# oxfordcontrol/Clarabel.rs

Hardware: AMD Instinct MI355X
Metric: IPM iterations/sec (KKT factor+solve) at n=10^6 SOCP, 1/2/4/8 GPUs (higher is better)
Workload: dtype f64

## Files before the change

### clarabel.rs_amd/csrc/bundle_ir.hip

```cpp
#include "dev_common.hpp"
#include "bundle_symv.hpp"
#include "ir_refine.hpp"
#include "grid_sync.hpp"

namespace chip {
namespace dev {

namespace {

constexpr int IR_SH_FWD = 3, IR_SH_BWD = 3, IR_SH_SYMV = 3;
constexpr int IR_RPT = 2;
constexpr int IR_FATCAP = 256;

template <bool FWDMODE, int SH, int RPT, int TW>
__device__ __forceinline__ void bundle_sweep_cols(const LdlView &v, const BundleView &bv, int b, double *xs,
                                                  const double *xt, double *tacc, int k, int *fat, int &nfat,
                                                  const double *__restrict__ dinv = nullptr) {
    constexpr int CH = RPT * TW;
    const int s0 = bv.bundle_ptr[b], nloc = bv.bundle_ptr[b + 1] - s0;
    const int *lv = bv.blvl + bv.blvl_ptr[b];
    const int nl = bv.blvl_ptr[b + 1] - bv.blvl_ptr[b] - 1;
    const int lane = threadIdx.x & 63, wv = threadIdx.x >> 6;
    if (FWDMODE && (int)threadIdx.x < 8) tacc[threadIdx.x] = 0.0;
    double tpart = 0.0;
// ... 174 lines not shown
    int i[FLAT_U], j[FLAT_U];
    double v[FLAT_U];
};
__device__ __forceinline__ void flat_batch_clear(FlatBatch &fb) {
#pragma unroll
    for (int u = 0; u < FLAT_U; ++u) fb.i[u] = -1, fb.j[u] = 0, fb.v[u] = 0.0;
}
template <bool FWDMODE, int TW>
__device__ __forceinline__ void flat_request_first(const LdlView &v, const int *lev_e, int nl, int dl, int tid, FlatBatch &fb) {
    int step = 0, base = 0, ee = 0;
    while (step < nl) {
        const int l = FWDMODE ? step : nl - 1 - step;
        base = lev_e[l];
        ee = lev_e[l + 1];
        if (base < ee) break;
        ++step;
    }
    if (step < nl) {
#pragma unroll
        for (int u = 0; u < FLAT_U; ++u) {
            const int t = base + u * TW + tid;
            const bool ok = t < ee;
            const int tc = ok ? t : ee - 1;
            const int ri = (int)v.Li16[tc + dl], rj = (int)v.Lj16[tc + dl];
            const double rv = v.Lx[tc];
            fb.i[u] = ok ? ri : -1;
            fb.j[u] = ok ? rj : 0;
            fb.v[u] = ok ? rv : 0.0;
        }
    } else {
        flat_batch_clear(fb);
    }
}
template <bool FWDMODE, int TW, bool HAVE_FIRST = true>
__device__ __forceinline__ void bundle_sweep_flat_ahead(const LdlView &v, double *xs, const double *xt, double *tacc, int k,
                                                        const int *lev_e, int dl, int nloc, int nl, const FlatBatch &first) {
    static_assert(TW != 512, "two batches in flight: not within the 80 registers of the 512-thread form");
    int tid = threadIdx.x;
    asm volatile("" : "+v"(tid));
    const int lane = tid & 63;
    if (FWDMODE && tid < 8) tacc[tid] = 0.0;
    double tpart = 0.0;
    int step = 0, base = 0, ee = 0;
    auto level_range = [&](int st_, int &eb_, int &ee_) {
        const int l = FWDMODE ? st_ : nl - 1 - st_;
        eb_ = lev_e[l];
        ee_ = lev_e[l + 1];
    };
    lds_barrier();
    while (step < nl) {
        level_range(step, base, ee);
        if (base < ee) break;
        ++step;
    }
    int ci[FLAT_U], cj[FLAT_U], ni[FLAT_U], nj[FLAT_U];
    double cv[FLAT_U], nv[FLAT_U];
    auto request = [&](int bs, int en, int *ii, int *jj, double *vv) {
#pragma unroll
        for (int u = 0; u < FLAT_U; ++u) {
            const int t = bs + u * TW + tid;
            const bool ok = t < en;
            ii[u] = ok ? (int)v.Li16[t + dl] : -1;
            jj[u] = ok ? (int)v.Lj16[t + dl] : 0;
            vv[u] = ok ? v.Lx[t] : 0.0;
        }
    };
    if (HAVE_FIRST) {
#pragma unroll
        for (int u = 0; u < FLAT_U; ++u) {
            ci[u] = first.i[u];
            cj[u] = first.j[u];
            cv[u] = first.v[u];
        }
    } else if (step < nl) {
        request(base, ee, ci, cj, cv);
    }
    while (step < nl) {
        int nstep = step, nbase = base + TW * FLAT_U, nee = ee;
        if (nbase >= nee) {
            nstep = step + 1;
            while (nstep < nl) {
                level_range(nstep, nbase, nee);
                if (nbase < nee) break;
                ++nstep;
            }
        }
        if (nstep < nl) request(nbase, nee, ni, nj, nv);
#pragma unroll
        for (int u = 0; u < FLAT_U; ++u) {
            const int i = ci[u];
            if (i < 0) continue;
            if (FWDMODE) {
                const double val = cv[u] * xs[cj[u]];
                if (i < nloc) atomicAdd(&xs[i], -val);
                else if (k == 1) tpart += val;
                else atomicAdd(&tacc[i - nloc], val);
            } else {
                atomicAdd(&xs[cj[u]], -(cv[u] * (i < nloc ? xs[i] : xt[i - nloc])));
            }
        }
        if (nstep != step) lds_barrier();
        step = nstep;
        base = nbase;
        ee = nee;
#pragma unroll
        for (int u = 0; u < FLAT_U; ++u) {
            ci[u] = ni[u];
            cj[u] = nj[u];
            cv[u] = nv[u];
        }
    }
    if (FWDMODE && k == 1) {
        tpart = wave_sum_all(tpart);
        if (lane == 0 && tpart != 0.0) atomicAdd(&tacc[0], tpart);
    }
    lds_barrier();
}

template <bool FWDMODE, int TW>
__device__ __forceinline__ void bundle_sweep_flat(const LdlView &v, const BundleView &bv, int b, double *xs,
                                                  const double *xt, double *tacc, int k, const int *lev_e, int dl = 0) {
    const int s0 = bv.bundle_ptr[b], nloc = bv.bundle_ptr[b + 1] - s0;
    const int nl = bv.blvl_ptr[b + 1] - bv.blvl_ptr[b] - 1;
    int tid = threadIdx.x;
    asm volatile("" : "+v"(tid));
    if (!FWDMODE)
        for (int i = tid; i < nloc; i += TW) xs[i] *= v.Dinv[s0 + i];
    if constexpr (TW != 512) {
        bundle_sweep_flat_ahead<FWDMODE, TW, false>(v, xs, xt, tacc, k, lev_e, dl, nloc, nl, FlatBatch{});
    } else {
        const int lane = tid & 63;
// ... 617 lines not shown
        if ((GR ? gfirst : blockIdx.x == 0) && tid < k) {
            ir_put(ir, ir.perm[topnode(tid)], st.curt[tid]);
            cur[topnode(tid)] = st.curt[tid];
        }
    }
    if (GR && gfirst && tid == 0) {
        __hip_atomic_store(gf.gcnt + grp * 32, 0, __ATOMIC_RELAXED, __HIP_MEMORY_SCOPE_AGENT);
        __hip_atomic_store(gf.gcnt + grp * 32 + 1, 0, __ATOMIC_RELAXED, __HIP_MEMORY_SCOPE_AGENT);
    }
    if (blockIdx.x == 0 && tid == 0) {
        ir.res[0] = ok ? 1 : -1;
        ir.res[1] = st.rounds;
        ir.res[3] = st.sel;
        pub[64] = st.normb;
        pub[65] = st.norme;
    }
    stamp();
    ir_grid_exit(ir.ctl, __builtin_amdgcn_readfirstlane(st.gen) + 1, G);
}


constexpr int IRS_NPT = 12;
__device__ __forceinline__ int opaque_tid() {
    int t = threadIdx.x;
    asm volatile("" : "+v"(t));
    return t;
}

template <int TW, int NPT, int NLP>
__device__ __forceinline__ void irs_symv(const LdlView &v, const IrView &ir, const int *runs, const double (&c)[NPT],
                                         bool keep_e, double *xs, double *red, double *tacc3, int k, int s0,
                                         int nloc, int nleaf, const double *xt, double *out_norm, double *out_share,
                                         int du, bool have_fl, int fl_b, int fl_e, bool next_fwd,
                                         const int *lev_e, int nl, int dl, FlatBatch &nextb) {
    double cl[NLP];
    const int *__restrict__ Up = v.Up;
    const unsigned short *__restrict__ Ucol16 = v.Ucol16, *__restrict__ Urow16 = v.Urow16;
    const double *__restrict__ Ux = v.Ux;
    const int tid = opaque_tid();
    auto xpos = [&](int t) { return t < nleaf ? t : nloc + (t - nleaf); };
    constexpr int LR = 4, LS = 3;
    static_assert(NLP % LR == 0 && NLP <= NPT, "leaf passes");
    int tb[LR], te[LR];
#pragma unroll
    for (int u = 0; u < LR; ++u) {
        const int i = tid + u * TW;
        tb[u] = i < nleaf ? Up[s0 + i] : 0;
        te[u] = i < nleaf ? Up[s0 + i + 1] : 0;
    }
    const int fb = have_fl ? fl_b : Up[s0 + nleaf], fe = have_fl ? fl_e : Up[s0 + nloc];
    {
        RunWalk rw{runs, 0};
        double bq[NPT];
#pragma unroll
        for (int u = 0; u < NPT; ++u) {
            const int i = tid + u * TW;
            bq[u] = (i >= nleaf && i < nloc) ? ir_rhs(ir, rw.orig(i)) : 0.0;
        }
        lds_barrier();
#pragma unroll
        for (int u = 0; u < NPT; ++u) {
            const int i = tid + u * TW;
            if (i >= nleaf && i < nloc) {
                xs[xpos(i - nleaf)] = c[u];
                xs[i] = bq[u];
            }
        }
// ... 7 lines not shown
    lds_barrier();
    RunWalk rl{runs, 0};
#pragma unroll
    for (int p = 0; p < NLP / LR; ++p) {
        if (p * LR * TW < nleaf) {
            int jj[LR][LS];
            double vv[LR][LS], bi[LR], acc[LR];
#pragma unroll
            for (int u = 0; u < LR; ++u) {
                const int i = (p * LR + u) * TW + tid;
                bi[u] = i < nleaf ? ir_rhs(ir, rl.orig(i)) : 0.0;
                acc[u] = 0.0;
#pragma unroll
                for (int q = 0; q < LS; ++q) {
                    const int t = tb[u] + q;
                    const bool ok = t < te[u];
                    jj[u][q] = ok ? (int)Ucol16[t + du] : -1;
                    vv[u][q] = ok ? Ux[t] : 0.0;
                }
            }
#pragma unroll
            for (int u = 0; u < LR; ++u) {
                const int i = (p * LR + u) * TW + tid;
                const double xi = cl[p * LR + u];
                auto apply = [&](int j, double val) {
                    if (j >= nloc) {
                        acc[u] += val * xt[j - nloc];
                        if (k == 1) tpart += val * xi;
                        else atomicAdd(&tacc3[j - nloc], val * xi);
                    } else if (j == i) {
                        acc[u] += val * xi;
                    } else {
                        acc[u] += val * xs[xpos(j - nleaf)];
                        atomicAdd(&xs[j], -(val * xi));
                    }
                };
#pragma unroll
                for (int q = 0; q < LS; ++q)
                    if (jj[u][q] >= 0) apply(jj[u][q], vv[u][q]);
                for (int t = tb[u] + LS; t < te[u]; ++t) apply((int)Ucol16[t + du], Ux[t]);
                if (i < nleaf) {
                    const double val = bi[u] - acc[u];
                    if (keep_e) cl[p * LR + u] = val;
                    if (val != val) nan = true;
                    else mleaf = fmax(mleaf, fabs(val));
                }
                const int in = i + LR * TW;
                tb[u] = in < nleaf ? Up[s0 + in] : 0;
                te[u] = in < nleaf ? Up[s0 + in + 1] : 0;
            }
        }
    }
    {
        int fi[FLAT_U], fj[FLAT_U], ni[FLAT_U], nj[FLAT_U];
        double fv[FLAT_U], nv[FLAT_U];
        auto request = [&](int bs, int *pi, int *pj, double *pv) {
#pragma unroll
            for (int u = 0; u < FLAT_U; ++u) {
                const int t = bs + u * TW + tid;
                const bool ok = t < fe;
                pi[u] = ok ? (int)Urow16[t + du] : -1;
                pj[u] = ok ? (int)Ucol16[t + du] : 0;
                pv[u] = ok ? Ux[t] : 0.0;
            }
        };
        if (fb < fe) request(fb, fi, fj, fv);
        for (int base = fb; base < fe; base += TW * FLAT_U) {
            if (base + TW * FLAT_U < fe) request(base + TW * FLAT_U, ni, nj, nv);
            else {
#pragma unroll
                for (int u = 0; u < FLAT_U; ++u) ni[u] = -1;
            }
#pragma unroll
            for (int u = 0; u < FLAT_U; ++u) {
                const int i = fi[u], j = fj[u];
                if (i < 0) continue;
                const double xi = xs[xpos(i - nleaf)];
                if (j >= nloc) {
                    atomicAdd(&xs[i], -(fv[u] * xt[j - nloc]));
                    if (k == 1) tpart += fv[u] * xi;
                    else atomicAdd(&tacc3[j - nloc], fv[u] * xi);
                } else if (j == i) {
                    atomicAdd(&xs[i], -(fv[u] * xi));
                } else {
                    atomicAdd(&xs[i], -(fv[u] * xs[xpos(j - nleaf)]));
                    atomicAdd(&xs[j], -(fv[u] * xi));
                }
            }
#pragma unroll
            for (int u = 0; u < FLAT_U; ++u) {
                fi[u] = ni[u];
                fj[u] = nj[u];
                fv[u] = nv[u];
            }
        }
    }
    if (next_fwd) flat_request_first<true, TW>(v, lev_e, nl, dl, tid, nextb);
    lds_barrier();
    double m = mleaf;
#pragma unroll
    for (int u = 0; u < NPT; ++u) {
        const int i = tid + u * TW;
        if (i >= nleaf && i < nloc) {
            const double val = xs[i];
            if (val != val) nan = true;
            else m = fmax(m, fabs(val));
        }
    }
    if (keep_e) {
#pragma unroll
        for (int u = 0; u < NLP; ++u)
            if (tid + u * TW < nleaf) xs[tid + u * TW] = cl[u];
    }
    symv_close<true>(m, nan, tpart, k, tid, tacc3, red, out_norm, out_share);
}

__device__ __forceinline__ void irs_flag_timeout(const IrView &ir) {
    ir.res[2] = 1;
    if (ir.res_host) ir.res_host[2] = 1;
}
template <int TW, int NLP>
__global__ __launch_bounds__(TW) __attribute__((amdgpu_waves_per_eu(4, 4)))
void k_bundle_irs(LdlView v, BundleView bv, FoldView fold, IrView ir) {
    constexpr int NPT = IRS_NPT;
    extern __shared__ __attribute__((aligned(16))) char smem[];
    double *xs = (double *)smem;
    __shared__ double red[16];
    __shared__ int lev_e[FLAT_MAXLEV + 1];
    __shared__ double tacc3[8];
    __shared__ IrState st;
    __shared__ int pat[2];
    __shared__ int hdr[12];
    const int nb = bv.nb, G = gridDim.x, b = blockIdx.x;
    int tid = threadIdx.x;
    const int k = fold.k;
    const bool folded = k > 0;
    const int NF = k ? fold.NF : ir.N;
    if (ir.test_drop && b == G - 1 && G > 1) return;
    const bool use_desc = (ir.sf_flags & IRS_F_DESC) != 0;
    const bool ahead = (ir.sf_flags & IRS_F_CHAINED) == 0;
    static_assert(IRS_DESC_RUNS == IR_MAXRUNS && IRS_DESC_LEVELS + 1 <= FLAT_MAXLEV + 1 && TW >= IRS_DESC_INTS, "IrsDesc");
    if (use_desc && tid < IRS_DESC_INTS) {
        constexpr int LEV0 = offsetof(IrsDesc, lev_e) / sizeof(int), RUN0 = offsetof(IrsDesc, runs) / sizeof(int);
        static_assert(LEV0 == 12 && offsetof(IrsDesc, dl) == 16, "IrsDesc: head of 12 ints");
        const int w = ((const int *)(ir.desc + b))[tid];
        if (tid < LEV0) hdr[tid] = w;
        else if (tid < RUN0) lev_e[tid - LEV0] = w;
        else st.runs[tid - RUN0] = w;
        if (tid == 4 || tid == 5) pat[tid - 4] = w;
    }
    int s0 = 0, nloc = 0, nleaf = 0, nl = 0;
    if (!use_desc) {
        s0 = bv.bundle_ptr[b], nloc = bv.bundle_ptr[b + 1] - s0;
        nleaf = bv.blvl[bv.blvl_ptr[b] + 1] - s0;
        nl = bv.blvl_ptr[b + 1] - bv.blvl_ptr[b] - 1;
    }
    double *pnb = ir.part;
    double *pn = pnb + nb;
    double *shf = pn + 2 * nb;
    double *shs = shf + (size_t)nb * k;
    double *pub = shs + 2 * (size_t)nb * k;
    if (tid == 0) {
        ir_verdict_init(st);
        st.par = 0;
        st.gen = 0;
        if (!use_desc) {
            pat[0] = ir.pat_off ? ir.pat_off[2 * b] : 0;
            pat[1] = ir.pat_off ? ir.pat_off[2 * b + 1] : 0;
        }
        if (b == 0) {
            ir.res[0] = 0;
            ir.res[2] = 0;
            if (ir.res_host) ir.res_host[0] = 0, ir.res_host[2] = 0;
        }
    }
    if (tid < 64) {
        st.ltt[tid] = 0.0;
        st.ktt[tid] = 0.0;
    }
    if (!use_desc) {
        const int r0 = ir.run_ptr[b], nruns = ir.run_ptr[b + 1] - r0;
        if (tid < 3 * nruns) st.runs[tid] = ir.runs[3 * r0 + tid];
        flat_level_table(v, bv, b, lev_e);
// ... 186 lines not shown
            c[u] = i < nloc ? ir_rhs(ir, rw.orig(i)) : 0.0;
        }
        if (ahead) {
            flat_request_first<true, TW>(v, lev_e, nl, __builtin_amdgcn_readfirstlane(pat[0]), opaque_tid(), fwdb);
            fwd_have = true;
        }
        double mx = 0.0;
        bool nan = false;
#pragma unroll
        for (int u = 0; u < NPT; ++u) {
            const int i = tid + u * TW;
            if (i < nloc) {
                xs[i] = c[u];
                if (ir.bp) ir.bp[s0 + i] = c[u];
                norm_take(c[u], mx, nan);
            }
        }
        mx = block_norm_or_nan(mx, nan, red);
        if (tid == 0) ir_store(&pnb[b], mx);
    }
    bool pending = false;
    double xk[NPT];
    bool xk_valid = false;
    bool spec_done = false;
    for (int round = 0;; ++round) {
        const int par = round & 1;
        asm volatile("" : "+v"(tid));
        __syncthreads();
        stamp();
        {
            const int dl = __builtin_amdgcn_readfirstlane(pat[0]);
            if (!fwd_have) flat_request_first<true, TW>(v, lev_e, nl, dl, opaque_tid(), fwdb);
            fwd_have = false;
            bundle_sweep_flat_ahead<true, TW>(v, xs, nullptr, st.tacc, k, lev_e, dl, nloc, nl, fwdb);
            flat_batch_clear(fwdb);
        }
        stamp();
        if (tid < k) ir_store(&shf[(size_t)b * k + tid], st.tacc[tid]);
        if (folded) {
            stamp();
            if (round == 0) load_top_constants();
            if (barrier(true, pending, par ^ 1, round == 1, true) == IR_TIMEOUT) {
                if (tid == 0) irs_flag_timeout(ir);
                return;
            }
            stamp();
            if (pending) {
                decide(round - 1, par ^ 1);
                pending = false;
                if (__builtin_amdgcn_readfirstlane(st.done)) break;
            }
            if (tid == 0) {
                ir_top_solve(k, [&](int i) { return (round == 0 ? st.btop[i] : st.rtop[i]) - st.pubv[i]; }, st.ltt, st.dinvt,
                             st.dxt);
                for (int i = 0; i < k; ++i) st.candt[i] = ir_top_cand(round, st.curt[i], st.dxt[i]);
            }
        }
        __syncthreads();
        stamp();
        {
            const int dl = __builtin_amdgcn_readfirstlane(pat[0]);
            if (!dinv_have) request_dinv();
            if (!bwd_have) flat_request_first<false, TW>(v, lev_e, nl, dl, opaque_tid(), bwdb);
            dinv_have = bwd_have = false;
            const int t_ = opaque_tid();
#pragma unroll
            for (int u = 0; u < NPT; ++u) {
// ... 40 lines not shown
            } else if (more_possible || !ir.spec_out) {
#pragma unroll
                for (int u = 0; u < NPT; ++u) {
                    const int i = tid + u * TW;
                    if (i < nloc) {
                        alt[s0 + i] = c[u];
                        if (xk_valid) cur[s0 + i] = xk[u];
                    }
                }
                xk_valid = false;
            } else {
                RunWalk rw{st.runs, 0};
#pragma unroll
                for (int u = 0; u < NPT; ++u) {
                    const int i = tid + u * TW;
                    if (i < nloc) ir_put(ir, rw.orig(i), c[u]);
                }
                spec_done = true;
            }
        }
        if (!ir.ir_enable) {
            double mx = 0.0;
            bool nan = false;
#pragma unroll
            for (int u = 0; u < NPT; ++u)
                if (tid + u * TW < nloc) norm_take(c[u], mx, nan);
            mx = block_norm_or_nan(mx, nan, red);
            if (tid == 0) ir_store(&pn[(size_t)par * nb + b], mx);
        } else {
            stamp();
            irs_symv<TW, NPT, NLP>(v, ir, st.runs, c, more_possible, xs, red, tacc3, k, s0, nloc, nleaf, st.candt,
                                   &pn[(size_t)par * nb + b], &shs[(size_t)par * nb * k + (size_t)b * k],
                                   __builtin_amdgcn_readfirstlane(pat[1]), use_desc, fl_b, fl_e,
                                   ahead && folded && more_possible, lev_e, nl, __builtin_amdgcn_readfirstlane(pat[0]), fwdb);
            fwd_have = ahead && folded && more_possible;
        }
        pending = true;
        if (folded && more_possible) continue;
        stamp();
        if (barrier(false, true, par, round == 0, false) == IR_TIMEOUT) {
            if (tid == 0) irs_flag_timeout(ir);
            return;
        }
        stamp();
        decide(round, par);
        pending = false;
        if (__builtin_amdgcn_readfirstlane(st.done)) break;
    }
    stamp();
    const int ok = __builtin_amdgcn_readfirstlane(st.ok);
    if (ok) {
        const bool accepted_last = __builtin_amdgcn_readfirstlane(st.accept) != 0;
        if (!(spec_done && accepted_last)) {
            const int tid = opaque_tid();
            const double *cur = __builtin_amdgcn_readfirstlane(st.sel) ? ir.xb : ir.xa;
            if (!xk_valid) {
#pragma unroll
                for (int u = 0; u < NPT; ++u) {
                    const int i = tid + u * TW;
                    xk[u] = i < nloc ? cur[s0 + i] : 0.0;
                }
            }
            RunWalk rw{st.runs, 0};
#pragma unroll
            for (int u = 0; u < NPT; ++u) {
                const int i = tid + u * TW;
                if (i < nloc) ir_put(ir, rw.orig(i), xk[u]);
// ... 120 lines not shown
```

### clarabel.rs_amd/csrc/capi.cpp

```cpp
#include <algorithm>
#include <cmath>
#include <cstdio>
#include <cstdlib>
#include <cstring>
#include <memory>

#include "batch_psd.hpp"
#include "engine.hpp"
#include "host_util.hpp"
#include "problem_update.hpp"
#include "../../include/clarabel_hip_testing.h"

using namespace chip;

namespace {

thread_local std::string g_last;

const i64 *as_i64(const uint64_t *p) { return reinterpret_cast<const i64 *>(p); }

void fill_info(const Engine &E, chip_info *info) {
    std::memset(info, 0, sizeof(*info));
    std::strncpy(info->name, "hip", sizeof(info->name) - 1);
    info->threads = 1;
    info->direct = 1;
    info->nnzA = E.nnzK;
    info->nnzL = E.nnzL;
    info->n = E.N;
    info->n_levels = E.tree_depth;
    info->amd_lnz = E.amd.lnz;
    info->amd_ndiv = E.amd.ndiv;
    info->amd_nmultsubs_ldl = E.amd.nmultsubs_ldl;
    info->regularize_count = E.last_regularize_count;
    info->positive_inertia = -1;
}

int count_positive(Engine &E, i64 *out) {
// ... 140 lines not shown

struct chip_kkt {
    KktLayout K;
    Engine E;
    int *mapHs = nullptr, *diag_full = nullptr, *mapP = nullptr, *mapA = nullptr;
    int nn_count = 0, zero_count = 0;
    int *nn_rows = nullptr, *nn_hsidx = nullptr, *zero_rows = nullptr;
    dev::SocView soc{};
    dev::Ns3View ns3{};
    dev::GpwView gpw{};
    std::vector<int> gpw_cone_index, gpw_state_off, gpw_dim1;
    dev::PsdView psd{};
    bool has_hostHs = false;
    double *d_s = nullptr, *d_z = nullptr, *d_w = nullptr, *d_lam = nullptr;
    double *d_rhs = nullptr, *d_lhs = nullptr;
    struct SolveVecs {
        double *bp = nullptr, *x = nullptr, *e = nullptr, *dx = nullptr;
        int last_ir = 0;
    } wk[2];
    double *d_tmp = nullptr;
    size_t tmp_len = 0;
    double last_eps = 0;
    bool scaling_pending_check = false;
    bool psd_rows_all_blocks = false;
    int scaling_gen = 0;
    bool x_holds_b = false;
    double static_diag_max = 0.0;
    const double *rhs_x = nullptr, *rhs_z = nullptr;
    bool rhs_deferred = false;
    int *ir_run_ptr = nullptr, *ir_runs = nullptr;
    bool ir_sf = false, bp_stale = false;
    std::vector<int> h_irs_desc;
    int *irs_desc = nullptr;
    bool irs_desc_shared = false;
#ifdef CHIP_TESTING
    std::vector<int> t_bundle_ptr, t_blvl_ptr, t_blvl, t_Lp, t_Up, t_run_ptr, t_runs, t_pat_off;
    std::vector<uint16_t> t_fu_rec, t_fr_rec;
    std::vector<int> t_fu_ptr, t_fr_desc, t_fr_ptr, t_fr_rptr, t_fu_lvl_ptr, t_fr_bdesc, t_fc_usr, t_fc_col, t_fc_sgn, t_fc_desc, t_fc_rec;
#endif
    int pend_update = 0;
    int pend_update_ok = 1;
    std::vector<int> pend_slots;
    struct FusedArgs {
        const double *rx, *rz;
        double *lx, *lz;
    } fused_args[Engine::IR_RING] = {};
    int fused_fallbacks = 0;
    #ifdef CHIP_TESTING
    bool ir_test_drop = switches().ir_test_drop;
#else
    static constexpr bool ir_test_drop = false;
#endif
    int world = 1;
    double *d_partial = nullptr;
    int partial_cap = 0;
    std::vector<double> h_partial;
};

extern "C" {

void chip_settings_default(chip_settings *s) {
    std::memset(s, 0, sizeof(*s));
    s->static_regularization_enable = 1;
    s->static_regularization_constant = 1e-8;
    s->static_regularization_proportional = 2.220446049250313e-16 * 2.220446049250313e-16;
    s->dynamic_regularization_enable = 1;
    s->dynamic_regularization_eps = 1e-13;
    s->dynamic_regularization_delta = 2e-7;
    s->iterative_refinement_enable = 1;
// ... 286 lines not shown
            int e = t + 1;
            while (e < s1 && pm[(size_t)e] == pm[(size_t)e - 1] + 1 && range_of(pm[(size_t)e]) == range_of(pm[(size_t)t])) e++;
            runs.push_back(t - s0);
            runs.push_back(pm[(size_t)t]);
            runs.push_back(e - t);
            t = e;
        }
        rp.push_back((int)(runs.size() / 3));
    }
}
static std::vector<int> irs_descriptors(const Symbolic &S, const std::vector<int> &rp, const std::vector<int> &runs,
                                        const std::vector<i32> *pat_off) {
    const int nb = S.bundle_ptr.empty() ? 0 : (int)S.bundle_ptr.size() - 1;
    std::vector<int> out;
    if (nb <= 0 || (int)rp.size() != nb + 1) return out;
    for (int b = 0; b < nb; b++)
        if (!dev::irs_desc_fits(S.blvl_ptr[(size_t)b + 1] - S.blvl_ptr[(size_t)b] - 1, rp[(size_t)b + 1] - rp[(size_t)b])) return out;
    out.assign((size_t)nb * dev::IRS_DESC_INTS, 0);
    for (int b = 0; b < nb; b++) {
        dev::IrsDesc d{};
        const i32 *lv = S.blvl.data() + S.blvl_ptr[(size_t)b];
        d.s0 = S.bundle_ptr[(size_t)b];
        d.nloc = S.bundle_ptr[(size_t)b + 1] - d.s0;
        d.nleaf = lv[1] - d.s0;
        d.nl = S.blvl_ptr[(size_t)b + 1] - S.blvl_ptr[(size_t)b] - 1;
        d.dl = pat_off ? (*pat_off)[2 * (size_t)b] : 0;
        d.du = pat_off ? (*pat_off)[2 * (size_t)b + 1] : 0;
        d.fb = S.Up[(size_t)(d.s0 + d.nleaf)];
        d.fe = S.Up[(size_t)(d.s0 + d.nloc)];
        d.nruns = rp[(size_t)b + 1] - rp[(size_t)b];
        for (int l = 0; l <= d.nl; l++) d.lev_e[l] = S.Lp[(size_t)lv[l]];
        std::copy_n(&runs[3 * (size_t)rp[(size_t)b]], 3 * (size_t)d.nruns, d.runs);
        std::memcpy(&out[(size_t)b * dev::IRS_DESC_INTS], &d, sizeof d);
    }
    return out;
}

int32_t chip_kkt_create(chip_kkt **out, int64_t n, int64_t m, const uint64_t *Pcolptr,
                        const uint64_t *Prowval, const double *Pnzval, const uint64_t *Acolptr,
                        const uint64_t *Arowval, const double *Anzval, int64_t ncones,
                        const int32_t *cone_tags, const int64_t *cone_dims, const int64_t *cone_dims2,
                        const double *cone_alphas_or_null, const chip_settings *settings,
                        const uint64_t *perm_or_null) {
    if (!out || n < 0 || m < 0 || !Pcolptr || !Acolptr) return fail(CHIP_ERR_ARG, "chip_kkt_create: bad argument");
    *out = nullptr;
#ifdef CHIP_TESTING
    create_count(0)++;
#endif
    switches_reload();
    chip_settings st;
    if (settings) st = *settings;
    else chip_settings_default(&st);
    std::unique_ptr<chip_kkt> h(new chip_kkt());
    KktLayout &K = h->K;
    i64 mm = 0;
    PhaseClock clk;
    clk.tag = "kkt_create";
    int rc = build_cone_specs(ncones, cone_tags, cone_dims, cone_dims2, K.cones, mm, K.p, K.nHs);
    if (rc) return CHIP_ERR_ARG;
    if (mm != m) return fail(CHIP_ERR_DIM, "cone dimensions do not add up to m");
    rc = assemble_kkt_triu(n, m, as_i64(Pcolptr), as_i64(Prowval), Pnzval, as_i64(Acolptr), as_i64(Arowval),
                           Anzval, K);
    if (rc) return rc;
    clk("KKT assembly");
    std::vector<i64> perm0;
    if (perm_or_null) perm0.assign(as_i64(perm_or_null), as_i64(perm_or_null) + K.N);
    Symbolic S;
    std::vector<i32> clique_of;
    {
        i32 g = 0;
        for (const ConeSpec &c : K.cones)
            if (!c.hs_diag && c.numel >= 16) {
                if (clique_of.empty()) clique_of.assign((size_t)K.N, -1);
                for (i64 r = 0; r < c.numel; r++) clique_of[(size_t)(n + c.start + r)] = g;
                g++;
            }
    }
    rc = analyse(K.N, K.colptr.data(), K.rowval.data(), K.dsigns.data(), perm0, st.amd_dense_scale, S, target_workgroups(st),
                 clique_of.empty() ? nullptr : &clique_of);
    if (rc) return rc;
    clk("analysis (total)");
    Engine &E = h->E;
    PatternShare pat;
    bool pat_cand = false;
    {
        const i32 nbun = S.bundle_ptr.empty() ? 0 : (i32)S.bundle_ptr.size() - 1;
        bool cand = !S.Li16.empty() && S.gf_ng == 0 && S.nfold >= 1 && nbun > 0;
        for (i32 b = 0; b < nbun && cand; b++) {
            const i32 s0 = S.bundle_ptr[(size_t)b], nloc = S.bundle_ptr[(size_t)b + 1] - s0;
            const i32 nleaf = S.blvl[(size_t)S.blvl_ptr[(size_t)b] + 1] - s0;
            cand = dev::irs_bundle_ok(nloc, nleaf, S.blvl_ptr[(size_t)b + 1] - S.blvl_ptr[(size_t)b] - 1, 1);
        }
        if (cand) {
            bundle_pattern_classes(S, pat);
            E.note_patterns(pat);
            clk("pattern classes");
        }
        pat_cand = cand;
    }
    const bool pat_shared = !pat.off.empty() && !pat.mismatches && !switches().no_shared_pattern;
    std::vector<int> run_ptr, runs;
    if (pat_cand) {
        bundle_perm_runs(S, K.n, K.m, run_ptr, runs);
        bool fit = true;
        for (size_t b = 0; b + 1 < run_ptr.size() && fit; b++) fit = run_ptr[b + 1] - run_ptr[b] <= dev::IRS_DESC_RUNS;
        if (fit) h->h_irs_desc = irs_descriptors(S, run_ptr, runs, pat_shared ? &pat.off : nullptr);
        clk("bundle descriptors");
    }
    if (st.device == CHIP_DEVICE_HOST_ONLY) {
#ifdef CHIP_TESTING
        if (pat_cand) {
            h->t_bundle_ptr = S.bundle_ptr, h->t_blvl_ptr = S.blvl_ptr, h->t_blvl = S.blvl;
            h->t_Lp = S.Lp, h->t_Up = S.Up, h->t_run_ptr = run_ptr, h->t_runs = runs;
            if (pat_shared) h->t_pat_off = pat.off;
        }
#endif
        E.init_host_only(S, st);
#ifdef CHIP_TESTING
        h->t_fu_lvl_ptr = S.blvl_ptr;
        h->t_fu_rec = std::move(S.fu_rec), h->t_fu_ptr = std::move(S.fu_ptr);
        h->t_fr_rec = std::move(S.fr_rec), h->t_fr_desc = std::move(S.fr_desc);
        h->t_fr_ptr = std::move(S.fr_ptr), h->t_fr_rptr = std::move(S.fr_rptr);
        h->t_fr_bdesc = std::move(S.fr_bdesc);
        h->t_fc_usr.assign(S.fc_usr.begin(), S.fc_usr.end()), h->t_fc_col.assign(S.fc_col.begin(), S.fc_col.end());
        h->t_fc_sgn.assign(S.fc_sgn.begin(), S.fc_sgn.end()), h->t_fc_rec.assign(S.fc_rec.begin(), S.fc_rec.end());
        h->t_fc_desc = std::move(S.fc_desc);
#endif
        *out = h.release();
        return CHIP_OK;
    }
    rc = E.init(S, st);
    if (rc) return rc;
    clk("engine init (uploads)");
    if (K.nnz) {
        rawvec<double> vx((size_t)K.nnz);
        run_threads(K.nnz >= (i64)1 << 22 ? host_threads() : 1, [&](int t, int TT) {
            for (i64 u = K.nnz * t / TT; u < K.nnz * (t + 1) / TT; u++) vx[(size_t)u] = K.nzval[(size_t)S.v2k[(size_t)u]];
        });
        CHIP_HIP(hipMemcpy(E.Kx, vx.data(), (size_t)K.nnz * sizeof(double), hipMemcpyHostToDevice));
    }
    const bigvec &k2v = S.k2v;
    auto narrow = [&k2v](const auto &v, size_t cnt) {
        rawvec<int> o(cnt);
// ... 214 lines not shown
    CHIP_HIP(hipMemset(st8, 0, (size_t)(sv.ncones ? sv.ncones : 1) * 8 * sizeof(double)));
    sv.eta = st8;
    sv.d = st8;
    sv.fail = &E.mb_dev->soc_fail;
    if ((rc = E.alloc(&h->d_rhs, (size_t)(n + m)))) return rc;
    if ((rc = E.alloc(&h->d_lhs, (size_t)(n + m)))) return rc;
    if ((rc = E.alloc(&h->wk[0].bp, (size_t)K.N))) return rc;
    if ((rc = E.alloc(&h->wk[0].x, (size_t)K.N))) return rc;
    if ((rc = E.alloc(&h->wk[0].e, (size_t)K.N))) return rc;
    if ((rc = E.alloc(&h->wk[0].dx, (size_t)K.N))) return rc;
    h->tmp_len = std::max<size_t>({(size_t)K.N, (size_t)K.nHs, nnzP, nnzA, 1});
    if ((rc = E.alloc(&h->d_tmp, h->tmp_len))) return rc;
    CHIP_HIP(hipMemset(h->wk[0].bp, 0, (size_t)(K.N ? K.N : 1) * sizeof(double)));
    if (E.ir_fused) {
        if (run_ptr.empty()) bundle_perm_runs(S, K.n, K.m, run_ptr, runs);
        const std::vector<int> &rp = run_ptr;
        if (!runs.empty() && (i64)(runs.size() / 3) * 64 <= (i64)E.NF) {
            if ((rc = E.upload(&h->ir_run_ptr, rp, rp.size()))) return rc;
            if ((rc = E.upload(&h->ir_runs, runs, runs.size()))) return rc;
            bool sf = E.gfold.ng == 0 && E.fold.k >= 1 && E.ir_tw == 256 && E.bundles.symv_split && E.bundles.nb == E.ir_grid &&
                      !switches().no_ir_sf && !switches().no_flat;
            for (int b = 0; b < E.bundles.nb && sf; b++) {
                const int s0 = S.bundle_ptr[(size_t)b], nloc = S.bundle_ptr[(size_t)b + 1] - s0;
                const int nleaf = S.blvl[(size_t)S.blvl_ptr[(size_t)b] + 1] - s0;
                const int nlev = S.blvl_ptr[(size_t)b + 1] - S.blvl_ptr[(size_t)b] - 1;
                sf = dev::irs_bundle_ok(nloc, nleaf, nlev, rp[(size_t)b + 1] - rp[(size_t)b]);
            }
            h->ir_sf = sf && dev::bundle_irs_capacity_ok(E.bundles);
            E.mb_mirror_on = h->ir_sf && E.fold.k == 1 && E.fast_prep_ok;
            if (h->ir_sf && !switches().no_shared_pattern && (rc = E.upload_patterns(pat))) return rc;
            if (h->ir_sf && !h->h_irs_desc.empty() && (E.pat_off != nullptr) == pat_shared &&
                (rc = E.upload(&h->irs_desc, h->h_irs_desc, h->h_irs_desc.size())))
                return rc;
            h->irs_desc_shared = pat_shared;
        }
    }
    clk("maps, cone tables");
    *out = h.release();
    return CHIP_OK;
}

void chip_kkt_destroy(chip_kkt *h) { delete h; }

int32_t chip_kkt_dims(const chip_kkt *h, int64_t out[8]) {
    if (!h) return CHIP_ERR_ARG;
    out[0] = h->K.n;
    out[1] = h->K.m;
    out[2] = h->K.p;
    out[3] = h->K.N;
    out[4] = h->K.nnz;
    out[5] = h->K.nHs;
    out[6] = h->E.NF;
    out[7] = h->E.nnzU;
    return CHIP_OK;
}
int32_t chip_kkt_degree(const chip_kkt *h, int64_t *degree) {
    if (!h || !degree) return CHIP_ERR_ARG;
    i64 d = 0;
    for (const ConeSpec &c : h->K.cones) {
        switch (c.tag) {
        case CHIP_CONE_ZERO: break;
        case CHIP_CONE_NONNEGATIVE: d += c.dim; break;
        case CHIP_CONE_SECONDORDER: d += 1; break;
        case CHIP_CONE_PSDTRIANGLE: d += c.dim; break;
        case CHIP_CONE_EXPONENTIAL:
        case CHIP_CONE_POWER: d += 3; break;
// ... 589 lines not shown
            return a && b_ && a < b_ + nb_ && b_ < a + na;
        };
        const size_t n = (size_t)h->K.n, m = (size_t)h->K.m;
        const int flags = (switches().irs_flags < 0 ? 3 : switches().irs_flags) & ~dev::IRS_F_DESC;
        ir.sf_flags = flags;
        ir.spec_out = (flags & 2) && !(overlap(lhsx_dev, n, ir.rx, n) || overlap(lhsx_dev, n, ir.rz, m) || overlap(lhsz_dev, m, ir.rx, n) ||
                        overlap(lhsz_dev, m, ir.rz, m));
    }
    h->bp_stale = ir.sf != 0;
    if ((rc0 = E.wait_for_exchange())) return rc0;
    h->fused_args[*slot] = {h->rhs_x, h->rhs_z, lhsx_dev, lhsz_dev};
    h->rhs_deferred = false;
    h->x_holds_b = false;
    E.prof_begin(PF_IR);
    int rc;
    if (step_kernel) {
        E.gstep.epoch += 1;
        dev::GStepView gsv = E.gstep;
        if (!E.gstep_vals_valid) gsv.gsl = gsv.gsu = nullptr;
        rc = dev::gstep_solve(E.stream, E.view(), E.bundles, ir, E.gfold, gsv);
    } else if (ir.sf) {
        dev::LdlView lv = E.view();
        ir.pat_off = nullptr;
        if (E.pat_off && !switches().no_shared_pattern) {
            lv.Li16 = E.pat_Li16;
            lv.Lj16 = E.pat_Lj16;
            lv.Ucol16 = E.pat_Ucol16;
            lv.Urow16 = E.pat_Urow16;
            ir.pat_off = E.pat_off;
        }
        if (h->irs_desc && !(ir.sf_flags & (dev::IRS_F_CHAINED)) && h->irs_desc_shared == (ir.pat_off != nullptr)) {
            ir.desc = (const dev::IrsDesc *)h->irs_desc;
            ir.sf_flags |= dev::IRS_F_DESC;
        }
        if (E.mirror_writes()) ir.res_host = E.mb_mirror->ring + 4 * *slot;
        rc = dev::bundle_ir(E.stream, lv, E.bundles, E.fold, ir, E.ir_grid, E.ir_tw, E.gfold);
    } else {
        rc = dev::bundle_ir(E.stream, E.view(), E.bundles, E.fold, ir, E.ir_grid, E.ir_tw, E.gfold);
    }
    E.prof_end(PF_IR);
    if (rc) return fail(CHIP_ERR_HIP, hip_err((hipError_t)rc, "fused solve launch"));
    E.note_mailbox_writer(ir.res_host != nullptr);
    if (dbg_all_on) {
        (void)hipStreamSynchronize(E.stream);
        std::vector<long long> t((size_t)E.ir_grid * 32);
        (void)hipMemcpy(t.data(), dbg_all_dev, t.size() * sizeof(long long), hipMemcpyDeviceToHost);
        const std::string &path = switches().ir_debug_file;
        if (FILE *f = std::fopen(path.empty() ? "/tmp/chip_ir_stamps.bin" : path.c_str(), "wb")) {
            const int g = E.ir_grid;
            std::fwrite(&g, sizeof(int), 1, f);
            std::fwrite(t.data(), sizeof(long long), t.size(), f);
            std::fclose(f);
        }
    } else if (dbg_on) {
        long long t[256];
        (void)hipStreamSynchronize(E.stream);
        (void)hipMemcpy(t, dbg_dev, sizeof(t), hipMemcpyDeviceToHost);
        for (int w = 0; w < 2; w++) {
            std::fprintf(stderr, "k_bundle_ir wg%d phases (us):", w);
            for (int i = 1; i < 64 && t[64 * w + i]; i++) std::fprintf(stderr, " %.1f", (t[64 * w + i] - t[64 * w + i - 1]) * 0.01);
            std::fprintf(stderr, "\n");
        }
    }
    return CHIP_OK;
}
constexpr int FUSED_TIMEOUT = -1000;
// ... 613 lines not shown
    else if (k == "gsweep_recoveries") *out = E.gs_recoveries;
    else if (k == "tri2_launches") *out = E.tri2_launches;
    else if (k == "dblk2_launches") *out = (double)E.dblk2_launches;
    else if (k == "dblk_blocks") *out = E.dblk.nblk;
    else if (k == "hs_direct_refactors") *out = (double)E.hs_direct_refactors;
    else if (k == "gsweep_levels") {
        int c = 0;
        for (const auto &r : E.gs_runs) c += r.nlev;
        *out = c;
    }
    else if (k == "pattern_classes") *out = E.pat_classes;
    else if (k == "pattern_index_bytes") *out = (double)E.pat_index_bytes;
    else if (k == "pattern_bundles") *out = E.pat_bundles;
    else if (k == "pattern_full_index_bytes") *out = (double)E.pat_full_bytes;
    else if (k == "pattern_verified_bundles") *out = E.pat_verified;
    else if (k == "pattern_mismatches") *out = E.pat_mismatches;
    else if (k == "pattern_shared_bundles")
        *out = (h->ir_sf && E.pat_off && !switches().no_shared_pattern) ? E.bundles.nb : 0;
    else if (k == "factor_runs") *out = E.fr_runs;
    else if (k == "factor_record_bundles") *out = E.fr_bundles;
    else if (k == "factor_classes") *out = E.fc_classes;
    else if (k == "factor_class_verified") *out = E.fc_verified;
    else if (k == "factor_class_mismatches") *out = E.fc_mismatches;
    else if (k == "factor_run_leftover") *out = E.fr_left;
    else if (k == "factor_run_max_leftover") *out = E.fr_max_left;
    else if (k == "factor_run_invalid") *out = E.fr_invalid;
    else if (k == "factor_run_kernel") *out = (E.fr_desc && E.factor_lds_doubles > 0 && !switches().no_factor_flat && !(E.gstep_factor_on && !switches().no_step_kernel)) ? 1 : 0;
    else if (k == "factor_records_on_device") *out = E.fu_rec ? 1 : 0;
    else if (k == "irs_desc_bundles") {
        const bool shared = E.pat_off && !switches().no_shared_pattern;
        const int flags = switches().irs_flags < 0 ? 3 : switches().irs_flags;
        *out = (h->ir_sf && h->irs_desc && !(flags & dev::IRS_F_CHAINED) && h->irs_desc_shared == shared) ? E.bundles.nb : 0;
    }
    else if (k == "mailbox_mirror_on") *out = E.mirror_writes() ? 1 : 0;
    else if (k == "mailbox_copies") *out = (double)E.mailbox_copies;
    else if (k == "mailbox_mirror_reads") *out = (double)E.mailbox_mirror_reads;
    else return fail(CHIP_ERR_ARG, "chip_debug_counter: unknown name");
    return CHIP_OK;
}
int32_t chip_debug_kkt_ints(const void *handle, const char *name, int64_t *len, int32_t *out) {
    const chip_kkt *h = (const chip_kkt *)handle;
    if (!h || !name || !len) return fail(CHIP_ERR_ARG, "chip_debug_kkt_ints: bad argument");
    const std::string k(name);
    const std::vector<int> *v = nullptr;
    if (k == "irs_desc") v = &h->h_irs_desc;
    else if (k == "bundle_ptr") v = &h->t_bundle_ptr;
    else if (k == "blvl_ptr") v = &h->t_blvl_ptr;
    else if (k == "blvl") v = &h->t_blvl;
    else if (k == "Lp") v = &h->t_Lp;
    else if (k == "Up") v = &h->t_Up;
    else if (k == "run_ptr") v = &h->t_run_ptr;
    else if (k == "runs") v = &h->t_runs;
    else if (k == "pat_off") v = &h->t_pat_off;
    else if (k == "factor_bundle_desc") v = &h->t_fr_bdesc;
    else if (k == "factor_class_usr") v = &h->t_fc_usr;
    else if (k == "factor_class_col") v = &h->t_fc_col;
    else if (k == "factor_class_sgn") v = &h->t_fc_sgn;
    else if (k == "factor_class_desc") v = &h->t_fc_desc;
    else if (k == "factor_class_rec") v = &h->t_fc_rec;
    else return fail(CHIP_ERR_ARG, "chip_debug_kkt_ints: unknown name");
    *len = (int64_t)v->size();
    if (out) std::copy(v->begin(), v->end(), out);
    return CHIP_OK;
}
int32_t chip_debug_kkt_factors(void *handle, double *Lx, double *D) {
    chip_kkt *h = (chip_kkt *)handle;
    if (!h) return fail(CHIP_ERR_ARG, "chip_debug_kkt_factors: bad argument");
    Engine &E = h->E;
    NEED_DEVICE(E);
    CHIP_HIP(hipSetDevice(E.device));
    CHIP_HIP(hipStreamSynchronize(E.stream));
    if (Lx && E.nnzL) CHIP_HIP(hipMemcpy(Lx, E.Lx, (size_t)E.nnzL * sizeof(double), hipMemcpyDeviceToHost));
    if (D && E.N) CHIP_HIP(hipMemcpy(D, E.D, (size_t)E.N * sizeof(double), hipMemcpyDeviceToHost));
    return CHIP_OK;
}
int32_t chip_debug_factor_updates(const void *handle, int32_t bundle, const char *what, int64_t *len, int32_t *out) {
    const chip_kkt *h = (const chip_kkt *)handle;
    if (!h || !what || !len) return fail(CHIP_ERR_ARG, "chip_debug_factor_updates: bad argument");
// ... 188 lines not shown
```

### clarabel.rs_amd/csrc/kernels.hpp

```cpp
#pragma once
#include <hip/hip_runtime.h>

#include <cstdint>

namespace chip {
namespace dev {

struct LdlView {
    int N;
    int nnzL;
    const int *Lp, *Li;
    const int *Rp, *Rcol, *Rpos;
    const int *Tpos;
    double *Lx, *Rx;
    double *D, *Dinv;
    const int8_t *dsigns;
    int *status;
    double reg_eps, reg_delta;
    const int *Up, *Ucol;
    const double *Ux;
    const double *eps_ptr;
    const unsigned long long *eps_slots;
    unsigned long long *eps_clear;
    double eps_c, eps_prop, eps_static_max;
// ... 92 lines not shown
int bundle_factor(hipStream_t s, const LdlView &v, const BundleView &bv, const FoldView &fold, int lds_doubles = 0);
bool bundle_factor_lds_ok(int lds_doubles);
bool bundle_factor_runs_ok(int max_nodes, int max_leftover, int max_levels);
struct MailboxMirror {
    const double *eps;
    const int *status, *soc_fail;
    double *h_eps;
    int *h_status, *h_soc_fail;
};
void fold_top_pivot(hipStream_t s, const LdlView &v, const FoldView &fold, const MailboxMirror &mm);
void bundle_fwd(hipStream_t s, const LdlView &v, const BundleView &bv, double *x, const FoldView &fold);
void fold_top_solve(hipStream_t s, const LdlView &v, const FoldView &fold, double *x);
void fold_top_residual(hipStream_t s, const FoldView &fold, const double *Sx, const double *x, const double *b,
                       double *e, unsigned long long *nrm, int *nan);
void bundle_bwd(hipStream_t s, const LdlView &v, const BundleView &bv, double *x, const double *addv);
void bundle_symv(hipStream_t s, const BundleView &bv, const int *Up, const int *Ucol, const double *Ux,
                 const double *x, const double *b, double *e, unsigned long long *nrm, int *nan, const FoldView &fold, hipEvent_t ev0 = nullptr, hipEvent_t ev1 = nullptr);
constexpr int IRS_DESC_LEVELS = 19;
constexpr int IRS_DESC_RUNS = 32;
struct alignas(16) IrsDesc {
    int s0, nloc, nleaf, nl;
    int dl, du;
    int fb, fe;
    int nruns, pad[3];
    int lev_e[IRS_DESC_LEVELS + 1];
    int runs[3 * IRS_DESC_RUNS];
};
static_assert(sizeof(IrsDesc) == 512, "IrsDesc: 128 ints, read as one dword per lane by two waves");
constexpr int IRS_DESC_INTS = (int)(sizeof(IrsDesc) / sizeof(int));
inline bool irs_desc_fits(int nlevels, int nruns) { return nlevels >= 1 && nlevels <= IRS_DESC_LEVELS && nruns >= 1 && nruns <= IRS_DESC_RUNS; }
constexpr int IRS_F_X0_REGS = 1;
constexpr int IRS_F_SPEC_OUT = 2;
constexpr int IRS_F_CHAINED = 4;
constexpr int IRS_F_DESC = 256;
struct IrView {
    const double *rx, *rz;
    int n, m, N;
    const int *perm;
    const int *run_ptr, *runs;
    double *bp;
    double *xa, *xb;
    union {
        double *ebuf;
        const int *pat_off;
        const IrsDesc *desc;
    };
    double *lhsx, *lhsz;
    double *part;
    int *ctl;
    int *res;
    double abstol, reltol, stopratio;
    int maxiter, ir_enable;
    long long *dbg;
    long long *dbg_all;
    int test_drop;
    int flat;
    int *rel;
    int epoch;
    int sf_flags;
    int spec_out;
    int sf;
    int *res_host;
};
int ir_rel_ints();
int ir_ctl_ints();
size_t ir_part_doubles(int nb, int k);
int bundle_ir_capacity(const BundleView &bv, int *tw);
int bundle_ir(hipStream_t s, const LdlView &v, const BundleView &bv, const FoldView &fold, const IrView &ir, int grid,
              int tw, const GFoldView &gf);
bool bundle_irs_capacity_ok(const BundleView &bv);
bool irs_bundle_ok(int nloc, int nleaf, int nlevels, int nruns);
void gfold_top_factor(hipStream_t s, const LdlView &v, const BundleView &bv, const GFoldView &gf);

constexpr int GS_MAXL = 14;
constexpr int GS_LST = GS_MAXL + 2;
constexpr int GS_DESC = 64;
constexpr int GS_GTOP = 152;
constexpr int GS_MV = 12;
struct GStepView {
    int lr, ur, nr;
    const int *desc;
    const int *gtop;
    const unsigned short *lsrc;
    const unsigned int *lij;
    const unsigned short *usrc;
    const unsigned int *uij;
    const unsigned short *ufs;
    double *gsl, *gsu;
    int *msg;
    int *lmsg;
    int *fmsg;
    int epoch;
    long long *dbg;
};
int gstep_solve_capacity(const BundleView &bv, const GStepView &gs);
// ... 231 lines not shown
```

Baseline: 1934.

## Privatize atomics to hot target rows in IR forward sweep and symv

Host analysis now picks, for each bundle level and for the symv residual, up to two local rows that receive many scatter updates (at least 64). The kernel accumulates updates to those rows in registers, reduces them across the wave, and issues one atomic per wave instead of one per element. This targets contention on shared-memory atomics at arrow-like dense rows in the SOCP KKT structure. The cost is extra compares and selects on every update, an extra shared array and a global load, and wave reductions at each level boundary.

```diff
diff --git a/clarabel.rs_amd/csrc/bundle_ir.hip b/clarabel.rs_amd/csrc/bundle_ir.hip
--- a/clarabel.rs_amd/csrc/bundle_ir.hip
+++ b/clarabel.rs_amd/csrc/bundle_ir.hip
@@ -230,15 +230,24 @@
         flat_batch_clear(fb);
     }
 }
-template <bool FWDMODE, int TW, bool HAVE_FIRST = true>
+template <bool FWDMODE, int TW, bool HAVE_FIRST = true, bool HOT = false>
 __device__ __forceinline__ void bundle_sweep_flat_ahead(const LdlView &v, double *xs, const double *xt, double *tacc, int k,
-                                                        const int *lev_e, int dl, int nloc, int nl, const FlatBatch &first) {
+                                                        const int *lev_e, int dl, int nloc, int nl, const FlatBatch &first,
+                                                        const int *hotl = nullptr) {
     static_assert(TW != 512, "two batches in flight: not within the 80 registers of the 512-thread form");
+    static_assert(!HOT || FWDMODE, "hot targets: the forward sweep's rows");
     int tid = threadIdx.x;
     asm volatile("" : "+v"(tid));
     const int lane = tid & 63;
     if (FWDMODE && tid < 8) tacc[tid] = 0.0;
     double tpart = 0.0;
+    double hacc0 = 0.0, hacc1 = 0.0;
+    int h0 = 0xFFFF, h1 = 0xFFFF;
+    auto hot_of = [&](int st_) {
+        const unsigned w = (unsigned)__builtin_amdgcn_readfirstlane(hotl[st_ < IRS_DESC_LEVELS ? st_ : IRS_HOT_INTS - 1]);
+        h0 = (int)(w & 0xFFFFu);
+        h1 = (int)(w >> 16);
+    };
     int step = 0, base = 0, ee = 0;
     auto level_range = [&](int st_, int &eb_, int &ee_) {
         const int l = FWDMODE ? st_ : nl - 1 - st_;
@@ -273,6 +282,8 @@
     } else if (step < nl) {
         request(base, ee, ci, cj, cv);
     }
+    if constexpr (HOT)
+        if (step < nl) hot_of(step);
     while (step < nl) {
         int nstep = step, nbase = base + TW * FLAT_U, nee = ee;
         if (nbase >= nee) {
@@ -290,11 +301,29 @@
             if (i < 0) continue;
             if (FWDMODE) {
                 const double val = cv[u] * xs[cj[u]];
+                if (HOT && (h0 & h1) != 0xFFFF) {
+                    const bool m0 = i == h0, m1 = i == h1;
+                    hacc0 += m0 ? val : 0.0;
+                    hacc1 += m1 ? val : 0.0;
+                    if (m0 || m1) continue;
+                }
                 if (i < nloc) atomicAdd(&xs[i], -val);
                 else if (k == 1) tpart += val;
                 else atomicAdd(&tacc[i - nloc], val);
             } else {
                 atomicAdd(&xs[cj[u]], -(cv[u] * (i < nloc ? xs[i] : xt[i - nloc])));
+            }
+        }
+        if constexpr (HOT) {
+            if (nstep != step) {
+                if ((h0 & h1) != 0xFFFF) {
+                    hacc0 = wave_sum_all(hacc0);
+                    hacc1 = wave_sum_all(hacc1);
+                    if (lane == 0 && h0 < nloc) atomicAdd(&xs[h0], -hacc0);
+                    if (lane == 0 && h1 < nloc) atomicAdd(&xs[h1], -hacc1);
+                    hacc0 = hacc1 = 0.0;
+                }
+                if (nstep < nl) hot_of(nstep);
             }
         }
         if (nstep != step) lds_barrier();
@@ -978,7 +1007,10 @@
                                          bool keep_e, double *xs, double *red, double *tacc3, int k, int s0,
                                          int nloc, int nleaf, const double *xt, double *out_norm, double *out_share,
                                          int du, bool have_fl, int fl_b, int fl_e, bool next_fwd,
-                                         const int *lev_e, int nl, int dl, FlatBatch &nextb) {
+                                         const int *lev_e, int nl, int dl, FlatBatch &nextb, int hotw) {
+    const int hc0 = hotw & 0xFFFF, hc1 = (int)((unsigned)hotw >> 16);
+    const bool hot_on = (hc0 & hc1) != 0xFFFF;
+    double hacc0 = 0.0, hacc1 = 0.0;
     double cl[NLP];
     const int *__restrict__ Up = v.Up;
     const unsigned short *__restrict__ Ucol16 = v.Ucol16, *__restrict__ Urow16 = v.Urow16;
@@ -1052,7 +1084,15 @@
                         acc[u] += val * xi;
                     } else {
                         acc[u] += val * xs[xpos(j - nleaf)];
-                        atomicAdd(&xs[j], -(val * xi));
+                        const double upd = val * xi;
+                        bool hit = false;
+                        if (hot_on) {
+                            const bool m0 = j == hc0, m1 = j == hc1;
+                            hacc0 += m0 ? upd : 0.0;
+                            hacc1 += m1 ? upd : 0.0;
+                            hit = m0 || m1;
+                        }
+                        if (!hit) atomicAdd(&xs[j], -upd);
                     }
                 };
 #pragma unroll
@@ -1104,7 +1144,15 @@
                     atomicAdd(&xs[i], -(fv[u] * xi));
                 } else {
                     atomicAdd(&xs[i], -(fv[u] * xs[xpos(j - nleaf)]));
-                    atomicAdd(&xs[j], -(fv[u] * xi));
+                    const double upd = fv[u] * xi;
+                    bool hit = false;
+                    if (hot_on) {
+                        const bool m0 = j == hc0, m1 = j == hc1;
+                        hacc0 += m0 ? upd : 0.0;
+                        hacc1 += m1 ? upd : 0.0;
+                        hit = m0 || m1;
+                    }
+                    if (!hit) atomicAdd(&xs[j], -upd);
                 }
             }
 #pragma unroll
@@ -1114,6 +1162,12 @@
                 fv[u] = nv[u];
             }
         }
+    }
+    if (hot_on) {
+        hacc0 = wave_sum_all(hacc0);
+        hacc1 = wave_sum_all(hacc1);
+        if ((tid & 63) == 0 && hc0 < nloc) atomicAdd(&xs[hc0], -hacc0);
+        if ((tid & 63) == 0 && hc1 < nloc) atomicAdd(&xs[hc1], -hacc1);
     }
     if (next_fwd) flat_request_first<true, TW>(v, lev_e, nl, dl, tid, nextb);
     lds_barrier();
@@ -1151,6 +1205,7 @@
     __shared__ IrState st;
     __shared__ int pat[2];
     __shared__ int hdr[12];
+    __shared__ int hotw[IRS_HOT_INTS];
     const int nb = bv.nb, G = gridDim.x, b = blockIdx.x;
     int tid = threadIdx.x;
     const int k = fold.k;
@@ -1169,6 +1224,9 @@
         else st.runs[tid - RUN0] = w;
         if (tid == 4 || tid == 5) pat[tid - 4] = w;
     }
+    static_assert(TW >= IRS_DESC_INTS + IRS_HOT_INTS, "hot targets: read by the lanes behind the record's");
+    if (tid >= IRS_DESC_INTS && tid < IRS_DESC_INTS + IRS_HOT_INTS)
+        hotw[tid - IRS_DESC_INTS] = ir.hot ? ir.hot[(size_t)b * IRS_HOT_INTS + (tid - IRS_DESC_INTS)] : -1;
     int s0 = 0, nloc = 0, nleaf = 0, nl = 0;
     if (!use_desc) {
         s0 = bv.bundle_ptr[b], nloc = bv.bundle_ptr[b + 1] - s0;
@@ -1421,7 +1479,7 @@
             const int dl = __builtin_amdgcn_readfirstlane(pat[0]);
             if (!fwd_have) flat_request_first<true, TW>(v, lev_e, nl, dl, opaque_tid(), fwdb);
             fwd_have = false;
-            bundle_sweep_flat_ahead<true, TW>(v, xs, nullptr, st.tacc, k, lev_e, dl, nloc, nl, fwdb);
+            bundle_sweep_flat_ahead<true, TW, true, true>(v, xs, nullptr, st.tacc, k, lev_e, dl, nloc, nl, fwdb, hotw);
             flat_batch_clear(fwdb);
         }
         stamp();
@@ -1528,7 +1586,8 @@
             irs_symv<TW, NPT, NLP>(v, ir, st.runs, c, more_possible, xs, red, tacc3, k, s0, nloc, nleaf, st.candt,
                                    &pn[(size_t)par * nb + b], &shs[(size_t)par * nb * k + (size_t)b * k],
                                    __builtin_amdgcn_readfirstlane(pat[1]), use_desc, fl_b, fl_e,
-                                   ahead && folded && more_possible, lev_e, nl, __builtin_amdgcn_readfirstlane(pat[0]), fwdb);
+                                   ahead && folded && more_possible, lev_e, nl, __builtin_amdgcn_readfirstlane(pat[0]), fwdb,
+                                   __builtin_amdgcn_readfirstlane(hotw[IRS_HOT_RESID]));
             fwd_have = ahead && folded && more_possible;
         }
         pending = true;
diff --git a/clarabel.rs_amd/csrc/capi.cpp b/clarabel.rs_amd/csrc/capi.cpp
--- a/clarabel.rs_amd/csrc/capi.cpp
+++ b/clarabel.rs_amd/csrc/capi.cpp
@@ -3,6 +3,7 @@
 #include <cstdio>
 #include <cstdlib>
 #include <cstring>
+#include <map>
 #include <memory>
 
 #include "batch_psd.hpp"
@@ -209,9 +210,12 @@
     bool ir_sf = false, bp_stale = false;
     std::vector<int> h_irs_desc;
     int *irs_desc = nullptr;
+    std::vector<int> h_irs_hot;
+    int *irs_hot = nullptr;
     bool irs_desc_shared = false;
 #ifdef CHIP_TESTING
     std::vector<int> t_bundle_ptr, t_blvl_ptr, t_blvl, t_Lp, t_Up, t_run_ptr, t_runs, t_pat_off;
+    std::vector<int> t_hot_bundle_ptr, t_hot_blvl_ptr, t_hot_blvl;
     std::vector<uint16_t> t_fu_rec, t_fr_rec;
     std::vector<int> t_fu_ptr, t_fr_desc, t_fr_ptr, t_fr_rptr, t_fu_lvl_ptr, t_fr_bdesc, t_fc_usr, t_fc_col, t_fc_sgn, t_fc_desc, t_fc_rec;
 #endif
@@ -564,6 +568,67 @@
         for (int l = 0; l <= d.nl; l++) d.lev_e[l] = S.Lp[(size_t)lv[l]];
         std::copy_n(&runs[3 * (size_t)rp[(size_t)b]], 3 * (size_t)d.nruns, d.runs);
         std::memcpy(&out[(size_t)b * dev::IRS_DESC_INTS], &d, sizeof d);
+    }
+    return out;
+}
+static std::vector<int> irs_hot_targets(const Symbolic &S, const std::vector<i32> *pat_off) {
+    const int nb = S.bundle_ptr.empty() ? 0 : (int)S.bundle_ptr.size() - 1;
+    std::vector<int> out;
+    if (nb <= 0 || S.Li16.empty() || S.Ucol16.empty()) return out;
+    out.assign((size_t)nb * dev::IRS_HOT_INTS, -1);
+    std::vector<int> cnt;
+    std::map<std::pair<i32, i32>, int> first_of_class;
+    for (int b = 0; b < nb; b++) {
+        const i32 s0 = S.bundle_ptr[(size_t)b], nloc = S.bundle_ptr[(size_t)b + 1] - s0;
+        const i32 *lv = S.blvl.data() + S.blvl_ptr[(size_t)b];
+        const int nl = S.blvl_ptr[(size_t)b + 1] - S.blvl_ptr[(size_t)b] - 1;
+        if (nl > dev::IRS_DESC_LEVELS || nloc >= 0xFFFF) return std::vector<int>();
+        int *row = &out[(size_t)b * dev::IRS_HOT_INTS];
+        if (pat_off) {
+            const auto key = std::make_pair((*pat_off)[2 * (size_t)b], (*pat_off)[2 * (size_t)b + 1]);
+            const auto it = first_of_class.find(key);
+            if (it != first_of_class.end()) {
+                std::copy_n(&out[(size_t)it->second * dev::IRS_HOT_INTS], dev::IRS_HOT_INTS, row);
+                continue;
+            }
+            first_of_class.emplace(key, b);
+        }
+        cnt.assign((size_t)nloc, 0);
+        std::vector<i32> touched;
+        auto pick = [&]() {
+            i32 best[dev::IRS_HOT_MAX] = {-1, -1};
+            std::sort(touched.begin(), touched.end());
+            for (i32 t : touched) {
+                if (cnt[(size_t)t] < dev::IRS_HOT_MIN) continue;
+                if (best[0] < 0 || cnt[(size_t)t] > cnt[(size_t)best[0]]) best[1] = best[0], best[0] = t;
+                else if (best[1] < 0 || cnt[(size_t)t] > cnt[(size_t)best[1]]) best[1] = t;
+            }
+            for (i32 t : touched) cnt[(size_t)t] = 0;
+            touched.clear();
+            const unsigned lo = best[0] < 0 ? 0xFFFFu : (unsigned)best[0], hi = best[1] < 0 ? 0xFFFFu : (unsigned)best[1];
+            return (int)(lo | hi << 16);
+        };
+        auto add = [&](i32 t) {
+            if (cnt[(size_t)t]++ == 0) touched.push_back(t);
+        };
+        for (int l = 0; l < nl; l++) {
+            for (i32 t = S.Lp[(size_t)lv[l]]; t < S.Lp[(size_t)lv[l + 1]]; t++)
+                if ((i32)S.Li16[(size_t)t] < nloc) add((i32)S.Li16[(size_t)t]);
+            row[l] = pick();
+        }
+        for (i32 i = 0; i < nloc; i++)
+            for (i32 t = S.Up[(size_t)(s0 + i)]; t < S.Up[(size_t)(s0 + i + 1)]; t++) {
+                const i32 j = (i32)S.Ucol16[(size_t)t];
+                if (j < nloc && j != i) add(j);
+            }
+        row[dev::IRS_HOT_RESID] = pick();
+    }
+    for (int b = 0; b < nb; b++) {
+        const unsigned nloc = (unsigned)(S.bundle_ptr[(size_t)b + 1] - S.bundle_ptr[(size_t)b]);
+        for (int w = 0; w < dev::IRS_HOT_INTS; w++) {
+            const unsigned x = (unsigned)out[(size_t)b * dev::IRS_HOT_INTS + w], lo = x & 0xFFFFu, hi = x >> 16;
+            if ((lo != 0xFFFFu && lo >= nloc) || (hi != 0xFFFFu && hi >= nloc)) return std::vector<int>();
+        }
     }
     return out;
 }
@@ -614,10 +679,11 @@
     clk("analysis (total)");
     Engine &E = h->E;
     PatternShare pat;
-    bool pat_cand = false;
+    bool pat_cand = false, arrow = false;
     {
         const i32 nbun = S.bundle_ptr.empty() ? 0 : (i32)S.bundle_ptr.size() - 1;
         bool cand = !S.Li16.empty() && S.gf_ng == 0 && S.nfold >= 1 && nbun > 0;
+        arrow = cand;
         for (i32 b = 0; b < nbun && cand; b++) {
             const i32 s0 = S.bundle_ptr[(size_t)b], nloc = S.bundle_ptr[(size_t)b + 1] - s0;
             const i32 nleaf = S.blvl[(size_t)S.blvl_ptr[(size_t)b] + 1] - s0;
@@ -639,8 +705,13 @@
         if (fit) h->h_irs_desc = irs_descriptors(S, run_ptr, runs, pat_shared ? &pat.off : nullptr);
         clk("bundle descriptors");
     }
+    if (arrow) {
+        h->h_irs_hot = irs_hot_targets(S, pat_shared ? &pat.off : nullptr);
+        clk("hot targets");
+    }
     if (st.device == CHIP_DEVICE_HOST_ONLY) {
 #ifdef CHIP_TESTING
+        if (arrow) h->t_hot_bundle_ptr = S.bundle_ptr, h->t_hot_blvl_ptr = S.blvl_ptr, h->t_hot_blvl = S.blvl;
         if (pat_cand) {
             h->t_bundle_ptr = S.bundle_ptr, h->t_blvl_ptr = S.blvl_ptr, h->t_blvl = S.blvl;
             h->t_Lp = S.Lp, h->t_Up = S.Up, h->t_run_ptr = run_ptr, h->t_runs = runs;
@@ -921,6 +992,7 @@
             if (h->ir_sf && !h->h_irs_desc.empty() && (E.pat_off != nullptr) == pat_shared &&
                 (rc = E.upload(&h->irs_desc, h->h_irs_desc, h->h_irs_desc.size())))
                 return rc;
+            if (h->irs_desc && !h->h_irs_hot.empty() && (rc = E.upload(&h->irs_hot, h->h_irs_hot, h->h_irs_hot.size()))) return rc;
             h->irs_desc_shared = pat_shared;
         }
     }
@@ -1576,6 +1648,7 @@
         if (h->irs_desc && !(ir.sf_flags & (dev::IRS_F_CHAINED)) && h->irs_desc_shared == (ir.pat_off != nullptr)) {
             ir.desc = (const dev::IrsDesc *)h->irs_desc;
             ir.sf_flags |= dev::IRS_F_DESC;
+            if (!(ir.sf_flags & dev::IRS_F_NO_HOT)) ir.hot = h->irs_hot;
         }
         if (E.mirror_writes()) ir.res_host = E.mb_mirror->ring + 4 * *slot;
         rc = dev::bundle_ir(E.stream, lv, E.bundles, E.fold, ir, E.ir_grid, E.ir_tw, E.gfold);
@@ -2255,6 +2328,12 @@
         const int flags = switches().irs_flags < 0 ? 3 : switches().irs_flags;
         *out = (h->ir_sf && h->irs_desc && !(flags & dev::IRS_F_CHAINED) && h->irs_desc_shared == shared) ? E.bundles.nb : 0;
     }
+    else if (k == "irs_hot_bundles") {
+        const bool shared = E.pat_off && !switches().no_shared_pattern;
+        const int flags = switches().irs_flags < 0 ? 3 : switches().irs_flags;
+        *out = (h->ir_sf && h->irs_desc && h->irs_hot && !(flags & (dev::IRS_F_CHAINED | dev::IRS_F_NO_HOT)) && h->irs_desc_shared == shared)
+                   ? E.bundles.nb : 0;
+    }
     else if (k == "mailbox_mirror_on") *out = E.mirror_writes() ? 1 : 0;
     else if (k == "mailbox_copies") *out = (double)E.mailbox_copies;
     else if (k == "mailbox_mirror_reads") *out = (double)E.mailbox_mirror_reads;
@@ -2267,6 +2346,10 @@
     const std::string k(name);
     const std::vector<int> *v = nullptr;
     if (k == "irs_desc") v = &h->h_irs_desc;
+    else if (k == "irs_hot") v = &h->h_irs_hot;
+    else if (k == "irs_hot_bundle_ptr") v = &h->t_hot_bundle_ptr;
+    else if (k == "irs_hot_blvl_ptr") v = &h->t_hot_blvl_ptr;
+    else if (k == "irs_hot_blvl") v = &h->t_hot_blvl;
     else if (k == "bundle_ptr") v = &h->t_bundle_ptr;
     else if (k == "blvl_ptr") v = &h->t_blvl_ptr;
     else if (k == "blvl") v = &h->t_blvl;
diff --git a/clarabel.rs_amd/csrc/kernels.hpp b/clarabel.rs_amd/csrc/kernels.hpp
--- a/clarabel.rs_amd/csrc/kernels.hpp
+++ b/clarabel.rs_amd/csrc/kernels.hpp
@@ -148,7 +148,11 @@
 constexpr int IRS_F_X0_REGS = 1;
 constexpr int IRS_F_SPEC_OUT = 2;
 constexpr int IRS_F_CHAINED = 4;
+constexpr int IRS_F_NO_HOT = 8;
 constexpr int IRS_F_DESC = 256;
+constexpr int IRS_HOT_MIN = 64, IRS_HOT_MAX = 2;
+constexpr int IRS_HOT_INTS = 32, IRS_HOT_RESID = IRS_DESC_LEVELS;
+static_assert(IRS_HOT_RESID < IRS_HOT_INTS && IRS_HOT_MAX == 2, "hot targets: two 16-bit ids per word");
 struct IrView {
     const double *rx, *rz;
     int n, m, N;
@@ -177,6 +181,7 @@
     int spec_out;
     int sf;
     int *res_host;
+    const int *hot;
 };
 int ir_rel_ints();
 int ir_ctl_ints();
```

After: 1945, median of 6. Within noise of the previous version (+0.6%).
